# microsoft/AI2BMD

Measured on NVIDIA H100. Metric: MD steps/sec, higher is better.
Workload: dtype f32

## Files before the change

ai2bmd_b200/csrc/engine.cu:

```cuda
#include <cuda_runtime.h>
#include <cxxabi.h>

#include <algorithm>
#include <atomic>
#include <cmath>
#include <cstdarg>
#include <cstdio>
#include <cstdlib>
#include <cstring>
#include <mutex>
#include <string>
#include <vector>

#include "../../include/visnet_b200.h"
#include "k_edge.cuh"
#include "k_caph.cuh"
#include "k_comm.cuh"
#include "k_edge_tc.cuh"
#include "k_graph_embed.cuh"
#include <nvtx3/nvToolsExt.h>
#include "k_head.cuh"
#include "k_md.cuh"
#include "k_nonbonded.cuh"
#include "k_node.cuh"
// ... 572 lines not shown
    a.tile_rows = h->tile_rows;
    const int rows = h->tc_rows;
    const int tiles = (h->ws.Ecap + h->tile_rows - 1) / h->tile_rows;
    const int blocks = std::max(1, std::min(tiles, h->sm_count));
    if (rows == 32) Lc.launch(edge_fwd_tc_kernel<32>, dim3(blocks), dim3(TC2_THREADS), TC_SMEM_BYTES, a);
    else if (rows == 64) Lc.launch(edge_fwd_tc_kernel<64>, dim3(blocks), dim3(TC2_THREADS), TC_SMEM_BYTES, a);
    else if (rows == 96) Lc.launch(edge_fwd_tc_kernel<96>, dim3(blocks), dim3(TC2_THREADS), TC_SMEM_BYTES, a);
    else Lc.launch(edge_fwd_tc_kernel<128>, dim3(blocks), dim3(TC2_THREADS), TC_SMEM_BYTES, a);
    Lc.check();
}

void edge_fwd(Launcher& Lc, int l) {
    if (Lc.h->edge_tc & 1) { launch_edge_fwd_tc(Lc, l); return; }
    if (Lc.h->te_fwd == 64) launch_edge_fwd<64, 8>(Lc, l, 2);
    else launch_edge_fwd<32, 8>(Lc, l, 4);
}
void launch_edge_bwd_tc(Launcher& Lc, int l) {
    vb_handle* h = Lc.h;
    EdgeTcArgs a{};
    a.layer = l; a.mw = h->mw; a.ws = h->ws;
    const LayerW& lw = h->mw.layer[l];
    const size_t chunk = 4 * 8192;
    const bool upd = l < L - 1;
    int n = 0;
    a.jobs[n++] = TcJob{lw.tcWsN, 0};
    a.jobs[n++] = TcJob{lw.tcWsN + chunk, 1};
    a.jobs[n++] = TcJob{lw.tcW1N + chunk, 0};
    a.jobs[n++] = TcJob{lw.tcW1N, 1};
    if (upd) a.jobs[n++] = TcJob{lw.tcW1N + 2 * chunk, 1};
    a.njobs = n;
    a.tl = h->timeline ? h->d_tl + (size_t)(L + l) * TC_TL_SLOTS : nullptr;
    a.tile_rows = h->tile_rows;
    const int rows = h->tc_rows;
    const int tiles = (h->ws.Ecap + h->tile_rows - 1) / h->tile_rows;
    const int blocks = std::max(1, std::min(tiles, h->sm_count));
    if (rows == 32) Lc.launch(edge_bwd_tc_kernel<32>, dim3(blocks), dim3(TC2_THREADS), TC_SMEM_BYTES, a);
    else if (rows == 64) Lc.launch(edge_bwd_tc_kernel<64>, dim3(blocks), dim3(TC2_THREADS), TC_SMEM_BYTES, a);
    else if (rows == 96) Lc.launch(edge_bwd_tc_kernel<96>, dim3(blocks), dim3(TC2_THREADS), TC_SMEM_BYTES, a);
    else Lc.launch(edge_bwd_tc_kernel<128>, dim3(blocks), dim3(TC2_THREADS), TC_SMEM_BYTES, a);
    Lc.check();
}

void edge_bwd(Launcher& Lc, int l) {
    if (Lc.h->edge_tc & 2) { launch_edge_bwd_tc(Lc, l); return; }
    if (Lc.h->te_bwd == 64) launch_edge_bwd<64, 8>(Lc, l, 1);
    else launch_edge_bwd<32, 8>(Lc, l, 2);
}

void node_tc_common(const vb_handle* h, NodeTcArgs& a, int k) {
    a.layer = k; a.mw = h->mw; a.ws = h->ws;
    a.tx = (h->ws.N + TC_TE - 1) / TC_TE;
    a.tv = (3 * h->ws.N + TC_TE - 1) / TC_TE;
    a.njx = 3; a.njv = 5; a.jx = 1; a.jv = 1;
}
void node_tc_jobs(TcJob* jobs, const float* img, int n) {
    for (int c = 0; c < n; c++) jobs[c] = TcJob{img + (size_t)c * 4 * 8192, 0};
// ... 2789 lines not shown
```

ai2bmd_b200/csrc/k_edge_tc.cuh:

```cuda
#pragma once
#include "k_edge.cuh"
#include "tc_common.cuh"

namespace vb {

constexpr int TC_TE = 128;
constexpr int TC_STAGES = 2;
constexpr int TC_MAX_STAGES = 3;
constexpr int TC_SLABS = D / tc::SLAB_K;
static_assert((TC_SLABS & (TC_SLABS - 1)) == 0, "tc_slab rotates the slab order with a mask: TC_SLABS must be a power of two");
constexpr int TC_MAXJOBS = 12;
constexpr int TC_LT = D + LDS_PAD;
typedef float TcRow[TC_LT];

struct TcJob {
    const float* img;
    int accumulate;
};

struct TcShared {
    alignas(1024) uint8_t ring[TC_STAGES][tc::STAGE_BYTES];
    alignas(16) float tile[TC_TE][TC_LT];
    alignas(16) float abuf[TC_TE][TC_LT];
    EdgeMeta<TC_TE> meta;
// ... 39 lines not shown

constexpr int TC2_CWARPS = 16;
constexpr int TC2_CTHREADS = TC2_CWARPS * 32;
constexpr int TC2_THREADS = TC2_CTHREADS;
constexpr int TC2_NGRP = TC2_CTHREADS / D;

struct EdgeTcArgs {
    int layer;
    ModelW mw;
    Workspace ws;
    TcJob jobs[TC_MAXJOBS];
    int njobs;
    int tile_rows;
    unsigned long long* tl;
};
constexpr int TC_TL_SLOTS = 64;
#define TC_TL(k) do { if (a.tl != nullptr && blockIdx.x == 0 && it == 0 && threadIdx.x == 0) a.tl[k] = (unsigned long long)clock64(); } while (0)

__device__ __forceinline__ void csync() { asm volatile("bar.sync 1, %0;" ::"n"(TC2_CTHREADS) : "memory"); }

constexpr int TC2_WS_THREADS = TC2_CTHREADS / 2;
__device__ __forceinline__ bool tc2_is_mma_warp(int warp) { return ((warp >> 2) & 1) == 0; }
__device__ __forceinline__ void gather_sync() { asm volatile("bar.sync 2, %0;" ::"n"(TC2_WS_THREADS) : "memory"); }
__device__ __forceinline__ void handoff_arrive(int id) { asm volatile("bar.arrive %0, %1;" ::"r"(id), "n"(TC2_CTHREADS) : "memory"); }
__device__ __forceinline__ void handoff_wait(int id) { asm volatile("bar.sync %0, %1;" ::"r"(id), "n"(TC2_CTHREADS) : "memory"); }

template <int ROWS>
struct TcRing {
    static constexpr int NS = tc_nstages(ROWS);
    int next = 0;
};

template <int ROWS>
__device__ __forceinline__ void tc2_setup(TcShared& sh, const TcRing<ROWS>&, const TcJob* jobs, int njobs, int ntiles) {
    constexpr int NS = TcRing<ROWS>::NS;
    if (threadIdx.x == 0) {
        for (int s = 0; s < NS; s++) { tc::mbar_init(&sh.b_full[s], 1); sh.released[s] = 0; }
        tc::mbar_init(&sh.b_tile, TC2_CWARPS);
        sh.jobs = jobs; sh.njobs = njobs; sh.nslabs = ntiles * njobs * TC_SLABS;
        tc::fence_barrier_init();
    }
    __syncthreads();
    if (threadIdx.x == 0)
        for (int k = 0; k < NS; k++) tc_issue<NS>(sh, k);
}

// ... 221 lines not shown
    float* __restrict__ Fout = upd ? ws.F[l + 1] : nullptr;
    const float* __restrict__ QKV = ws.QKV[l];
    const float* __restrict__ VN = ws.VN[l];
    const float* __restrict__ TU = ws.TU[l];
    float* __restrict__ P1 = ws.P1[l];
    float* __restrict__ SP = ws.SP[l];
    float* __restrict__ ATT = ws.ATT[l];
    for (int it = 0; it < my_tiles; it++) {
        const uint32_t tpar = (uint32_t)(it & 1);
        const int e0 = ((int)blockIdx.x + it * (int)gridDim.x) * trows;
        const int nvalid = min(trows, E - e0);
        {
            constexpr int RW = ROWS / TC2_CWARPS;
            const int w0 = warp * RW, wn = max(0, min(RW, nvalid - w0));
            if (lane == 0) {
                if (wn > 0) tc::mbar_arrive_expect_tx(&sh.b_tile, (uint32_t)wn * D * 4);
                else tc::mbar_arrive(&sh.b_tile);
            }
            __syncwarp();
            if (lane < wn) tc::tma_load_1d(&sh.abuf[w0 + lane][0], Fin + (size_t)(e0 + w0 + lane) * D, D * 4, &sh.b_tile);
        }
        load_edge_meta<TC_TE, TC2_CTHREADS>(sh.meta, ws, e0, nvalid);
        if constexpr (SMALL) {
            enum : int { H_DK = 3, H_ATT, H_DV, H_F, H_M, H_EU };
            TcRow* const xb = tc_aux(sh);
            csync();
            if (tc2_is_mma_warp(warp)) {
                tc::mbar_wait(&sh.b_tile, tpar);
                TC_TL(2);
                tc2_mma<ROWS, true>(sh, ring, sh.abuf, acc, a.jobs[J_DK].accumulate, warp, lane, nvalid);
                tc2_acc_to(sh.tile, acc, warp, lane, nvalid);
                handoff_arrive(H_DK);
                TC_TL(4);
                tc2_mma<ROWS, true>(sh, ring, sh.abuf, acc, a.jobs[J_DV].accumulate, warp, lane, nvalid);
                TC_TL(7);
                handoff_wait(H_ATT);
                tc2_acc_to(xb, acc, warp, lane, nvalid);
                handoff_arrive(H_DV);
                TC_TL(8);
                if (upd) {
                    tc2_mma<ROWS, true>(sh, ring, sh.abuf, acc, a.jobs[J_F].accumulate, warp, lane, nvalid);
                    tc2_acc_to(sh.tile, acc, warp, lane, nvalid);
                    handoff_arrive(H_F);
                    TC_TL(11);
                }
                handoff_wait(H_M);
                TC_TL(3);
// ... 217 lines not shown
            TC_TL(15);
            if (threadIdx.x == 0 && it + 1 < my_tiles) {
                const int en = ((int)blockIdx.x + (it + 1) * (int)gridDim.x) * trows;
                tc::tma_prefetch_l2(Fin + (size_t)en * D, (uint32_t)min(trows, E - en) * D * 4);
            }
            tc2_mma(sh, ring, sh.abuf, acc, a.jobs[J_S2].accumulate, warp, lane, nvalid);
            TC_TL(16);
            csync();
            tc2_acc_to(sh.tile, acc, warp, lane, nvalid);
            csync();
            TC_TL(17);
            tc_fwd_s2(sh, ws, lw, SP, sh.tile, e0, nvalid, cch, grp, TC2_NGRP, bnd);
            TC_TL(18);
        }
        csync();
    }
    if (a.tl != nullptr && blockIdx.x == 0 && threadIdx.x == 0) a.tl[31] = (unsigned long long)clock64();
}

}

namespace vb {

template <int ROWS>
__global__ void __launch_bounds__(TC2_THREADS, 1) edge_bwd_tc_kernel(const __grid_constant__ EdgeTcArgs a) {
    pdl_entry();
    extern __shared__ __align__(1024) uint8_t dyn_raw[];
    TcShared& sh = *tc_shared_base(dyn_raw);
    const Workspace& ws = a.ws;
    const int l = a.layer;
    const bool upd = (l < L - 1);
    const int J_G3A = 0, J_G3B = 1, J_G4DV = 2, J_G4DK = 3, J_G4F = 4;
    const int J_LAST = upd ? J_G4F : J_G4DK;
    constexpr int RPW = ROWS / TC2_CWARPS;
    constexpr int RB4 = (RPW % 4 == 0) ? 4 : 2;
    constexpr bool SMALL = ROWS <= 64;
    constexpr int RBM = SMALL ? 2 : RB4;
    const int warp = threadIdx.x >> 5, lane = threadIdx.x & 31, col = lane * 4, hd = lane >> 2;
    const int E = ws.rowptr[ws.N];
    const int trows = min(ROWS, max(16, a.tile_rows));
    const int ntiles_total = (E + trows - 1) / trows;
    const int my_tiles = ((int)blockIdx.x < ntiles_total) ? (ntiles_total - (int)blockIdx.x + (int)gridDim.x - 1) / (int)gridDim.x : 0;
    if (a.tl != nullptr && blockIdx.x == 0 && threadIdx.x == 0) a.tl[0] = (unsigned long long)clock64();
    TcRing<ROWS> ring;
    tc2_setup(sh, ring, a.jobs, a.njobs, my_tiles);
    if (a.tl != nullptr && blockIdx.x == 0 && threadIdx.x == 0) a.tl[1] = (unsigned long long)clock64();

    float acc[32];
    const float* __restrict__ QKV = ws.QKV[l];
    const float* __restrict__ VN = ws.VN[l];
    const float* __restrict__ TU = ws.TU[l];
    const float* __restrict__ P1 = ws.P1[l];
    const float* __restrict__ SP = ws.SP[l];
    const float* __restrict__ ATT = ws.ATT[l];
    const int cch = threadIdx.x & (D - 1), grp = threadIdx.x >> 7;
    for (int it = 0; it < my_tiles; it++) {
        const int e0 = ((int)blockIdx.x + it * (int)gridDim.x) * trows;
        const int nvalid = min(trows, E - e0);
        const int rpw = (nvalid + TC2_CWARPS - 1) / TC2_CWARPS, r0 = warp * rpw;
        load_edge_meta<TC_TE, TC2_CTHREADS>(sh.meta, ws, e0, nvalid);
        csync();
// ... 15 lines not shown
                }
#pragma unroll
                for (int u = 0; u < RB4; u++) {
                    const int row = r0 + rb + u;
                    const bool mine = rb + u < rpw, ok = (mine && row < nvalid);
                    const size_t j3 = (size_t)sh.meta.src[row] * 3;
                    const float4 dd = sh.meta.d[row];
                    const float4 s1 = silu4(sp[u][0]), s2 = silu4(sp[u][1]);
                    const float4 gs1 = gM[u][0] * vn[u][0] + gM[u][1] * vn[u][1] + gM[u][2] * vn[u][2];
                    const float gx_ = warp_sum(hsum4(gM[u][0] * s2)), gy_ = warp_sum(hsum4(gM[u][1] * s2)), gz_ = warp_sum(hsum4(gM[u][2] * s2));
                    if (mine) {
                        st4(&sh.abuf[row][col], ok ? gs1 * dsilu4(sp[u][0]) : f4s(0.f));
                        st4(&sh.tile[row][col], ok ? (gM[u][0] * dd.x + gM[u][1] * dd.y + gM[u][2] * dd.z) * dsilu4(sp[u][1]) : f4s(0.f));
                        if (lane == 0) { sh.eacc[row][1] = gx_; sh.eacc[row][2] = gy_; sh.eacc[row][3] = gz_; }
                    }
                    if (ok) {
                        red4(ws.GVNMSG + (j3 + 0) * D + col, gM[u][0] * s1);
                        red4(ws.GVNMSG + (j3 + 1) * D + col, gM[u][1] * s1);
                        red4(ws.GVNMSG + (j3 + 2) * D + col, gM[u][2] * s1);
                    }
                }
            }
            TC_TL(3);
        } else {
#pragma unroll 1
            for (int rb = 0; rb < RPW; rb += RB4) {
                if (rb >= rpw) break;
                float4 sp[RB4], gM[RB4][3], vn[RB4][3];
#pragma unroll
                for (int u = 0; u < RB4; u++) {
                    const int row = r0 + rb + u;
                    const size_t e = (size_t)(e0 + ((rb + u < rpw && row < nvalid) ? row : 0));
                    const size_t i3 = (size_t)sh.meta.dst[row] * 3, j3 = (size_t)sh.meta.src[row] * 3;
                    sp[u] = ldg4(SP + e * 2 * D + col);
#pragma unroll
                    for (int s = 0; s < 3; s++) { gM[u][s] = ldg4(ws.GVEC + (i3 + s) * D + col); vn[u][s] = ldg4(VN + (j3 + s) * D + col); }
                }
#pragma unroll
                for (int u = 0; u < RB4; u++) {
                    const int row = r0 + rb + u;
                    const bool ok = (rb + u < rpw && row < nvalid);
                    const size_t j3 = (size_t)sh.meta.src[row] * 3;
                    const float4 s1 = silu4(sp[u]);
                    const float4 gs1 = gM[u][0] * vn[u][0] + gM[u][1] * vn[u][1] + gM[u][2] * vn[u][2];
                    if (rb + u < rpw) st4(&sh.abuf[row][col], ok ? gs1 * dsilu4(sp[u]) : f4s(0.f));
                    if (ok) {
// ... 1 lines not shown
                        red4(ws.GVNMSG + (j3 + 1) * D + col, gM[u][1] * s1);
                        red4(ws.GVNMSG + (j3 + 2) * D + col, gM[u][2] * s1);
                    }
                }
            }
            TC_TL(3);
#pragma unroll 4
            for (int r = 0; r < RPW; r++) {
                if (r >= rpw) break;
                const int row = r0 + r;
                const bool ok = (r < rpw && row < nvalid);
                const size_t e = (size_t)(e0 + (ok ? row : 0));
                const size_t i3 = (size_t)sh.meta.dst[row] * 3;
                const float4 dd = sh.meta.d[row];
                const float4 sp = ldg4(SP + e * 2 * D + D + col);
                const float4 s2 = silu4(sp);
                const float4 gM0 = ldg4(ws.GVEC + (i3 + 0) * D + col), gM1 = ldg4(ws.GVEC + (i3 + 1) * D + col),
                             gM2 = ldg4(ws.GVEC + (i3 + 2) * D + col);
                const float gx_ = warp_sum(hsum4(gM0 * s2)), gy_ = warp_sum(hsum4(gM1 * s2)), gz_ = warp_sum(hsum4(gM2 * s2));
                if (lane == 0) { sh.eacc[row][1] = gx_; sh.eacc[row][2] = gy_; sh.eacc[row][3] = gz_; }
                st4(&sh.tile[row][col], ok ? (gM0 * dd.x + gM1 * dd.y + gM2 * dd.z) * dsilu4(sp) : f4s(0.f));
            }
            TC_TL(5);
        }
        csync();
        tc2_mma(sh, ring, sh.abuf, acc, a.jobs[J_G3A].accumulate, warp, lane, nvalid);
        TC_TL(6);
        if constexpr (!SMALL) {
            tc2_tile_to_a(sh, nvalid);
            TC_TL(7);
        }
        tc2_mma(sh, ring, SMALL ? sh.tile : sh.abuf, acc, a.jobs[J_G3B].accumulate, warp, lane, nvalid);
        TC_TL(8);
        csync();
        tc2_acc_to(sh.tile, acc, warp, lane, nvalid);
        csync();
        TC_TL(9);
#pragma unroll 1
        for (int rb = 0; rb < RPW; rb += RBM) {
            if (rb >= rpw) break;
            float4 gxa[RBM], vjr[RBM], pdvr[RBM];
            float avr[RBM];
#pragma unroll
            for (int u = 0; u < RBM; u++) {
                const int row = r0 + rb + u;
                const size_t e = (size_t)(e0 + ((rb + u < rpw && row < nvalid) ? row : 0));
                gxa[u] = load_gxa(ws, (size_t)sh.meta.dst[row], col);
                vjr[u] = ldg4(QKV + (size_t)sh.meta.src[row] * 3 * D + 2 * D + col);
                pdvr[u] = ldg4(P1 + e * 3 * D + D + col);
                avr[u] = (rb + u < rpw && row < nvalid) ? __ldg(ATT + e * H + hd) : 0.f;
            }
#pragma unroll
            for (int u = 0; u < RBM; u++) {
                const int row = r0 + rb + u;
                const bool ok = (rb + u < rpw && row < nvalid);
                const size_t j = sh.meta.src[row];
                const float Ce = sh.meta.C[row];
                const float av = avr[u], sa = silu_(av), A = sa * Ce;
                const bool mine = rb + u < rpw;
                const float4 gm = mine ? ld4(&sh.tile[row][col]) + gxa[u] : f4s(0.f);
                const float4 dv = silu4(pdvr[u]);
                if (mine) st4(&sh.abuf[row][col], ok ? gm * vjr[u] * A * dsilu4(pdvr[u]) : f4s(0.f));
                const float gA = quad_sum(hsum4(gm * vjr[u] * dv));
                if (mine && (lane & 3) == 0) sh.gattn[row][hd] = gA * Ce * dsilu_(av);
                const float gc = warp_sum((lane & 3) == 0 ? gA * sa : 0.f);
                if (mine && lane == 0) sh.eacc[row][0] = gc;
                if (ok) red4(ws.GQKV + j * 3 * D + 2 * D + col, gm * dv * A);
            }
        }
        TC_TL(10);
        csync();
#pragma unroll 1
        for (int rb = 0; rb < RPW; rb += RB4) {
            if (rb >= rpw) break;
            float4 pdkr[RB4], qir[RB4], kjr[RB4];
#pragma unroll
            for (int u = 0; u < RB4; u++) {
                const int row = r0 + rb + u;
                const size_t e = (size_t)(e0 + ((rb + u < rpw && row < nvalid) ? row : 0));
                pdkr[u] = ldg4(P1 + e * 3 * D + col);
                qir[u] = ldg4(QKV + (size_t)sh.meta.dst[row] * 3 * D + col);
                kjr[u] = ldg4(QKV + (size_t)sh.meta.src[row] * 3 * D + D + col);
            }
#pragma unroll
            for (int u = 0; u < RB4; u++) {
                const int row = r0 + rb + u;
                const bool ok = (rb + u < rpw && row < nvalid);
                const size_t j = sh.meta.src[row];
                const float4 dk = silu4(pdkr[u]);
                const float gav = sh.gattn[row][hd];
                if (rb + u < rpw) st4(&sh.tile[row][col], ok ? qir[u] * kjr[u] * gav * dsilu4(pdkr[u]) : f4s(0.f));
                if (SMALL && rb + u < rpw) st4(&tc_aux(sh)[row][col], kjr[u] * dk * gav);
                if (ok) red4(ws.GQKV + j * 3 * D + D + col, qir[u] * dk * gav);
            }
        }
        TC_TL(12);
        csync();
        tc2_mma(sh, ring, sh.abuf, acc, a.jobs[J_G4DV].accumulate, warp, lane, nvalid);
        TC_TL(13);
        if constexpr (!SMALL) {
            tc2_tile_to_a(sh, nvalid);
            TC_TL(14);
            csync();
#pragma unroll 4
            for (int r = 0; r < RPW; r++) {
                if (r >= rpw) break;
                const int row = r0 + r;
                const size_t e = (size_t)(e0 + ((r < rpw && row < nvalid) ? row : 0));
                const float4 dk = silu4(ldg4(P1 + e * 3 * D + col));
                const float4 kj = ldg4(QKV + (size_t)sh.meta.src[row] * 3 * D + D + col);
                st4(&sh.tile[row][col], kj * dk * sh.gattn[row][hd]);
            }
            csync();
        }
        {
            const TcRow* const gqb = SMALL ? tc_aux(sh) : sh.tile;
            const int i_first = sh.meta.dst[0], i_last = sh.meta.dst[nvalid - 1];
            for (int i = i_first + grp; i <= i_last; i += TC2_NGRP) {
                const int q0 = ws.rowptr[i], q1 = ws.rowptr[i + 1];
                const int lo = max(q0, e0) - e0, hi = min(q1, e0 + nvalid) - e0;
                float gq = 0.f;
                for (int r = lo; r < hi; r++) gq += gqb[r][cch];
                if (q0 >= e0 && q1 <= e0 + nvalid) ws.GQKV[(size_t)i * 3 * D + cch] = gq;
                else atomicAdd(ws.GQKV + (size_t)i * 3 * D + cch, gq);
            }
        }
        TC_TL(15);
        if (upd) {
            TcRow* const gpfb = SMALL ? sh.abuf : sh.tile;
            csync();
#pragma unroll 1
            for (int rb = 0; rb < RPW; rb += 2) {
                if (rb >= rpw) break;
                float4 gfr[2], pfr[2], tir[2][3], ujr[2][3];
#pragma unroll
                for (int u = 0; u < 2; u++) {
                    const int row = r0 + rb + u;
                    const bool ok = (rb + u < rpw && row < nvalid);
                    const size_t e = (size_t)(e0 + (ok ? row : 0));
                    const size_t i3 = (size_t)sh.meta.dst[row] * 3, j3 = (size_t)sh.meta.src[row] * 3;
                    gfr[u] = ok ? ld4(ws.GF + e * D + col) : f4s(0.f);
                    pfr[u] = ldg4(P1 + e * 3 * D + 2 * D + col);
#pragma unroll
                    for (int s = 0; s < 3; s++) {
                        tir[u][s] = ldg4(TU + (i3 + s) * 2 * D + col);
                        ujr[u][s] = ldg4(TU + (j3 + s) * 2 * D + D + col);
                    }
                }
#pragma unroll
                for (int u = 0; u < 2; u++) {
                    const int row = r0 + rb + u;
                    const bool ok = (rb + u < rpw && row < nvalid);
                    const size_t e = (size_t)(e0 + (ok ? row : 0));
                    const size_t j3 = (size_t)sh.meta.src[row] * 3;
                    const float4 dd = sh.meta.d[row];
                    const float4 gfn = gfr[u], pf = pfr[u];
                    const float4 fp = silu4(pf);
                    const float dv3[3] = {dd.x, dd.y, dd.z};
                    const float4 a1 = tir[u][0] * dd.x + tir[u][1] * dd.y + tir[u][2] * dd.z;
                    const float4 a2 = ujr[u][0] * dd.x + ujr[u][1] * dd.y + ujr[u][2] * dd.z;
                    float4 w1[3], w2[3];
#pragma unroll
                    for (int s = 0; s < 3; s++) { w1[s] = tir[u][s] - a1 * dv3[s]; w2[s] = ujr[u][s] - a2 * dv3[s]; }
                    const float4 wdot = w1[0] * w2[0] + w1[1] * w2[1] + w1[2] * w2[2];
                    const float4 gwd = gfn * fp;
                    if (rb + u < rpw) {
                        st4(&gpfb[row][col], gfn * wdot * dsilu4(pf));
                        if (SMALL) st4(&tc_aux(sh)[row][col], gwd);
                    }
                    const float4 c1 = gwd * (w2[0] * dd.x + w2[1] * dd.y + w2[2] * dd.z);
                    const float4 c2 = gwd * (w1[0] * dd.x + w1[1] * dd.y + w1[2] * dd.z);
                    float gdl[3];
                    float4 gu[3];
#pragma unroll
                    for (int s = 0; s < 3; s++) {
                        const float4 gw1 = gwd * w2[s], gw2 = gwd * w1[s];
                        gu[s] = gw2 - c2 * dv3[s];
                        gdl[s] = warp_sum(hsum4(tir[u][s] * c1 + a1 * gw1 + ujr[u][s] * c2 + a2 * gw2));
                    }
                    if (lane == 0 && rb + u < rpw) { sh.eacc[row][1] -= gdl[0]; sh.eacc[row][2] -= gdl[1]; sh.eacc[row][3] -= gdl[2]; }
                    if (ok) {
                        red4(ws.GTU + (j3 + 0) * 2 * D + D + col, gu[0]);
                        red4(ws.GTU + (j3 + 1) * 2 * D + D + col, gu[1]);
                        red4(ws.GTU + (j3 + 2) * 2 * D + D + col, gu[2]);
                    }
                    (void)e;
                }
            }
            TC_TL(16);
            csync();
            tc2_mma(sh, ring, SMALL ? sh.tile : sh.abuf, acc, a.jobs[J_G4DK].accumulate, warp, lane, nvalid);
            TC_TL(17);
            if constexpr (!SMALL) {
                tc2_tile_to_a(sh, nvalid);
                TC_TL(18);
                csync();
#pragma unroll 4
                for (int r = 0; r < RPW; r++) {
                    if (r >= rpw) break;
                    const int row = r0 + r;
                    const bool ok = (r < rpw && row < nvalid);
                    const size_t e = (size_t)(e0 + (ok ? row : 0));
                    const float4 gfn = ok ? ld4(ws.GF + e * D + col) : f4s(0.f);
                    st4(&sh.tile[row][col], gfn * silu4(ldg4(P1 + e * 3 * D + 2 * D + col)));
                }
                csync();
            }
            {
                const TcRow* const gwb = SMALL ? tc_aux(sh) : sh.tile;
                const int i_first = sh.meta.dst[0], i_last = sh.meta.dst[nvalid - 1];
                for (int i = i_first + grp; i <= i_last; i += TC2_NGRP) {
                    const int q0 = ws.rowptr[i], q1 = ws.rowptr[i + 1];
                    const int lo = max(q0, e0) - e0, hi = min(q1, e0 + nvalid) - e0;
                    float gt0 = 0.f, gt1 = 0.f, gt2 = 0.f;
                    auto term = [&](int r, float u0, float u1, float u2) {
                        const float4 dd = sh.meta.d[r];
                        const float gw = gwb[r][cch];
                        const float a2 = u0 * dd.x + u1 * dd.y + u2 * dd.z;
                        const float w20 = u0 - a2 * dd.x, w21 = u1 - a2 * dd.y, w22 = u2 - a2 * dd.z;
                        const float wd = w20 * dd.x + w21 * dd.y + w22 * dd.z;
                        gt0 += gw * (w20 - wd * dd.x);
                        gt1 += gw * (w21 - wd * dd.y);
                        gt2 += gw * (w22 - wd * dd.z);
                    };
                    int r = lo;
                    for (; r + 4 <= hi; r += 4) {
                        float u[4][3];
#pragma unroll
                        for (int q = 0; q < 4; q++) {
                            const size_t j3 = (size_t)sh.meta.src[r + q] * 3;
                            u[q][0] = __ldg(TU + (j3 + 0) * 2 * D + D + cch);
                            u[q][1] = __ldg(TU + (j3 + 1) * 2 * D + D + cch);
                            u[q][2] = __ldg(TU + (j3 + 2) * 2 * D + D + cch);
                        }
#pragma unroll
                        for (int q = 0; q < 4; q++) term(r + q, u[q][0], u[q][1], u[q][2]);
                    }
                    for (; r < hi; r++) {
                        const size_t j3 = (size_t)sh.meta.src[r] * 3;
                        term(r, __ldg(TU + (j3 + 0) * 2 * D + D + cch), __ldg(TU + (j3 + 1) * 2 * D + D + cch),
                             __ldg(TU + (j3 + 2) * 2 * D + D + cch));
                    }
                    if (q0 >= e0 && q1 <= e0 + nvalid) {
                        ws.GTU[((size_t)i * 3 + 0) * 2 * D + cch] = gt0;
                        ws.GTU[((size_t)i * 3 + 1) * 2 * D + cch] = gt1;
                        ws.GTU[((size_t)i * 3 + 2) * 2 * D + cch] = gt2;
                    } else {
                        atomicAdd(ws.GTU + ((size_t)i * 3 + 0) * 2 * D + cch, gt0);
                        atomicAdd(ws.GTU + ((size_t)i * 3 + 1) * 2 * D + cch, gt1);
                        atomicAdd(ws.GTU + ((size_t)i * 3 + 2) * 2 * D + cch, gt2);
                    }
                }
            }
        }
        TC_TL(19);
        if (threadIdx.x < 3 && it + 1 < my_tiles) {
            const int en = ((int)blockIdx.x + (it + 1) * (int)gridDim.x) * trows;
            const uint32_t nn = (uint32_t)min(trows, E - en);
            if (threadIdx.x == 0) tc::tma_prefetch_l2(SP + (size_t)en * 2 * D, nn * 2 * D * 4);
            else if (threadIdx.x == 1) tc::tma_prefetch_l2(P1 + (size_t)en * 3 * D, nn * 3 * D * 4);
            else tc::tma_prefetch_l2(ATT + (size_t)en * H, nn * H * 4);
        }
        tc2_mma(sh, ring, (SMALL && !upd) ? sh.tile : sh.abuf, acc, a.jobs[J_LAST].accumulate, warp, lane, nvalid);
        TC_TL(20);
        if (!SMALL || !upd) csync();
        tc2_acc_to(sh.tile, acc, warp, lane, nvalid);
        csync();
        TC_TL(21);
#pragma unroll 4
        for (int r = 0; r < RPW; r++) {
            if (r >= rpw) break;
            const int row = r0 + r;
            if ((r < rpw && row < nvalid)) {
                float* g = ws.GF + (size_t)(e0 + row) * D + col;
                float4 v = ld4(&sh.tile[row][col]);
                if (upd) v = v + ld4(g);
                st4(g, v);
            }
        }
        if (threadIdx.x < nvalid) {
            float* ea = ws.eacc + (size_t)(e0 + threadIdx.x) * 4;
            st4(ea, ld4(ea) + ld4(&sh.eacc[threadIdx.x][0]));
        }
        TC_TL(22);
        csync();
    }
    if (a.tl != nullptr && blockIdx.x == 0 && threadIdx.x == 0) a.tl[31] = (unsigned long long)clock64();
}

// ... 2 lines not shown
```

Measured before the change: 1155.

## Warp-specialize small-tile edge backward kernel to overlap MMA with gather work

```diff
diff --git a/ai2bmd_b200/csrc/engine.cu b/ai2bmd_b200/csrc/engine.cu
--- a/ai2bmd_b200/csrc/engine.cu
+++ b/ai2bmd_b200/csrc/engine.cu
@@ -618,16 +618,18 @@
     const LayerW& lw = h->mw.layer[l];
     const size_t chunk = 4 * 8192;
     const bool upd = l < L - 1;
+    const int rows = h->tc_rows;
+    const bool pf_first = upd && rows <= 64;
     int n = 0;
     a.jobs[n++] = TcJob{lw.tcWsN, 0};
     a.jobs[n++] = TcJob{lw.tcWsN + chunk, 1};
-    a.jobs[n++] = TcJob{lw.tcW1N + chunk, 0};
+    if (pf_first) a.jobs[n++] = TcJob{lw.tcW1N + 2 * chunk, 0};
+    a.jobs[n++] = TcJob{lw.tcW1N + chunk, pf_first ? 1 : 0};
     a.jobs[n++] = TcJob{lw.tcW1N, 1};
-    if (upd) a.jobs[n++] = TcJob{lw.tcW1N + 2 * chunk, 1};
+    if (upd && !pf_first) a.jobs[n++] = TcJob{lw.tcW1N + 2 * chunk, 1};
     a.njobs = n;
     a.tl = h->timeline ? h->d_tl + (size_t)(L + l) * TC_TL_SLOTS : nullptr;
     a.tile_rows = h->tile_rows;
-    const int rows = h->tc_rows;
     const int tiles = (h->ws.Ecap + h->tile_rows - 1) / h->tile_rows;
     const int blocks = std::max(1, std::min(tiles, h->sm_count));
     if (rows == 32) Lc.launch(edge_bwd_tc_kernel<32>, dim3(blocks), dim3(TC2_THREADS), TC_SMEM_BYTES, a);
diff --git a/ai2bmd_b200/csrc/k_edge_tc.cuh b/ai2bmd_b200/csrc/k_edge_tc.cuh
--- a/ai2bmd_b200/csrc/k_edge_tc.cuh
+++ b/ai2bmd_b200/csrc/k_edge_tc.cuh
@@ -85,6 +85,7 @@
 constexpr int TC2_WS_THREADS = TC2_CTHREADS / 2;
 __device__ __forceinline__ bool tc2_is_mma_warp(int warp) { return ((warp >> 2) & 1) == 0; }
 __device__ __forceinline__ void gather_sync() { asm volatile("bar.sync 2, %0;" ::"n"(TC2_WS_THREADS) : "memory"); }
+__device__ __forceinline__ void mma_sync() { asm volatile("bar.sync 3, %0;" ::"n"(TC2_WS_THREADS) : "memory"); }
 __device__ __forceinline__ void handoff_arrive(int id) { asm volatile("bar.arrive %0, %1;" ::"r"(id), "n"(TC2_CTHREADS) : "memory"); }
 __device__ __forceinline__ void handoff_wait(int id) { asm volatile("bar.sync %0, %1;" ::"r"(id), "n"(TC2_CTHREADS) : "memory"); }
 
@@ -352,7 +353,7 @@
         }
         load_edge_meta<TC_TE, TC2_CTHREADS>(sh.meta, ws, e0, nvalid);
         if constexpr (SMALL) {
-            enum : int { H_DK = 3, H_ATT, H_DV, H_F, H_M, H_EU };
+            enum : int { H_DK = 4, H_ATT, H_DV, H_F, H_M, H_EU };
             TcRow* const xb = tc_aux(sh);
             csync();
             if (tc2_is_mma_warp(warp)) {
@@ -616,6 +617,202 @@
 
 namespace vb {
 
+
+template <int NR, int RB, class Wait>
+__device__ __forceinline__ void tc_bwd_gm(TcShared& sh, const Workspace& ws, const float* __restrict__ QKV,
+                                          const float* __restrict__ P1, const float* __restrict__ ATT, int e0, int nvalid,
+                                          int r0, int rpw, int lane, Wait&& wait) {
+    const int col = lane * 4, hd = lane >> 2;
+#pragma unroll 1
+    for (int rb = 0; rb < NR; rb += RB) {
+        if (rb >= rpw) break;
+        float4 gxa[RB], vjr[RB], pdvr[RB];
+        float avr[RB];
+#pragma unroll
+        for (int u = 0; u < RB; u++) {
+            const int row = r0 + rb + u;
+            const size_t e = (size_t)(e0 + ((rb + u < rpw && row < nvalid) ? row : 0));
+            gxa[u] = load_gxa(ws, (size_t)sh.meta.dst[row], col);
+            vjr[u] = ldg4(QKV + (size_t)sh.meta.src[row] * 3 * D + 2 * D + col);
+            pdvr[u] = ldg4(P1 + e * 3 * D + D + col);
+            avr[u] = (rb + u < rpw && row < nvalid) ? __ldg(ATT + e * H + hd) : 0.f;
+        }
+        if (rb == 0) wait();
+#pragma unroll
+        for (int u = 0; u < RB; u++) {
+            const int row = r0 + rb + u;
+            const bool ok = (rb + u < rpw && row < nvalid);
+            const size_t j = sh.meta.src[row];
+            const float Ce = sh.meta.C[row];
+            const float av = avr[u], sa = silu_(av), A = sa * Ce;
+            const bool mine = rb + u < rpw;
+            const float4 gm = mine ? ld4(&sh.tile[row][col]) + gxa[u] : f4s(0.f);
+            const float4 dv = silu4(pdvr[u]);
+            if (mine) st4(&sh.abuf[row][col], ok ? gm * vjr[u] * A * dsilu4(pdvr[u]) : f4s(0.f));
+            const float gA = quad_sum(hsum4(gm * vjr[u] * dv));
+            if (mine && (lane & 3) == 0) sh.gattn[row][hd] = gA * Ce * dsilu_(av);
+            const float gc = warp_sum((lane & 3) == 0 ? gA * sa : 0.f);
+            if (mine && lane == 0) sh.eacc[row][0] = gc;
+            if (ok) red4(ws.GQKV + j * 3 * D + 2 * D + col, gm * dv * A);
+        }
+    }
+}
+
+template <int NR, int RB, bool GQ>
+__device__ __forceinline__ void tc_bwd_gpdk(TcShared& sh, const Workspace& ws, const float* __restrict__ QKV,
+                                            const float* __restrict__ P1, int e0, int nvalid, int r0, int rpw, int lane) {
+    const int col = lane * 4, hd = lane >> 2;
+#pragma unroll 1
+    for (int rb = 0; rb < NR; rb += RB) {
+        if (rb >= rpw) break;
+        float4 pdkr[RB], qir[RB], kjr[RB];
+#pragma unroll
+        for (int u = 0; u < RB; u++) {
+            const int row = r0 + rb + u;
+            const size_t e = (size_t)(e0 + ((rb + u < rpw && row < nvalid) ? row : 0));
+            pdkr[u] = ldg4(P1 + e * 3 * D + col);
+            qir[u] = ldg4(QKV + (size_t)sh.meta.dst[row] * 3 * D + col);
+            kjr[u] = ldg4(QKV + (size_t)sh.meta.src[row] * 3 * D + D + col);
+        }
+#pragma unroll
+        for (int u = 0; u < RB; u++) {
+            const int row = r0 + rb + u;
+            const bool ok = (rb + u < rpw && row < nvalid);
+            const size_t j = sh.meta.src[row];
+            const float4 dk = silu4(pdkr[u]);
+            const float gav = sh.gattn[row][hd];
+            if (rb + u < rpw) st4(&sh.tile[row][col], ok ? qir[u] * kjr[u] * gav * dsilu4(pdkr[u]) : f4s(0.f));
+            if (GQ && rb + u < rpw) st4(&tc_aux(sh)[row][col], kjr[u] * dk * gav);
+            if (ok) red4(ws.GQKV + j * 3 * D + D + col, qir[u] * dk * gav);
+        }
+    }
+}
+
+template <int NR>
+__device__ __forceinline__ void tc_bwd_gpf(TcShared& sh, const Workspace& ws, const float* __restrict__ TU,
+                                           const float* __restrict__ P1, TcRow* dst, int e0, int nvalid, int r0, int rpw,
+                                           int lane) {
+    const int col = lane * 4;
+#pragma unroll 1
+    for (int rb = 0; rb < NR; rb += 2) {
+        if (rb >= rpw) break;
+        float4 gfr[2], pfr[2], tir[2][3], ujr[2][3];
+#pragma unroll
+        for (int u = 0; u < 2; u++) {
+            const int row = r0 + rb + u;
+            const bool ok = (rb + u < rpw && row < nvalid);
+            const size_t e = (size_t)(e0 + (ok ? row : 0));
+            const size_t i3 = (size_t)sh.meta.dst[row] * 3, j3 = (size_t)sh.meta.src[row] * 3;
+            gfr[u] = ok ? ld4(ws.GF + e * D + col) : f4s(0.f);
+            pfr[u] = ldg4(P1 + e * 3 * D + 2 * D + col);
+#pragma unroll
+            for (int s = 0; s < 3; s++) {
+                tir[u][s] = ldg4(TU + (i3 + s) * 2 * D + col);
+                ujr[u][s] = ldg4(TU + (j3 + s) * 2 * D + D + col);
+            }
+        }
+#pragma unroll
+        for (int u = 0; u < 2; u++) {
+            const int row = r0 + rb + u;
+            const bool ok = (rb + u < rpw && row < nvalid);
+            const size_t j3 = (size_t)sh.meta.src[row] * 3;
+            const float4 dd = sh.meta.d[row];
+            const float4 gfn = gfr[u], pf = pfr[u];
+            const float4 fp = silu4(pf);
+            const float dv3[3] = {dd.x, dd.y, dd.z};
+            const float4 a1 = tir[u][0] * dd.x + tir[u][1] * dd.y + tir[u][2] * dd.z;
+            const float4 a2 = ujr[u][0] * dd.x + ujr[u][1] * dd.y + ujr[u][2] * dd.z;
+            float4 w1[3], w2[3];
+#pragma unroll
+            for (int s = 0; s < 3; s++) { w1[s] = tir[u][s] - a1 * dv3[s]; w2[s] = ujr[u][s] - a2 * dv3[s]; }
+            const float4 wdot = w1[0] * w2[0] + w1[1] * w2[1] + w1[2] * w2[2];
+            const float4 gwd = gfn * fp;
+            if (rb + u < rpw) st4(&dst[row][col], gfn * wdot * dsilu4(pf));
+            const float4 c1 = gwd * (w2[0] * dd.x + w2[1] * dd.y + w2[2] * dd.z);
+            const float4 c2 = gwd * (w1[0] * dd.x + w1[1] * dd.y + w1[2] * dd.z);
+            float gdl[3];
+            float4 gu[3];
+#pragma unroll
+            for (int s = 0; s < 3; s++) {
+                const float4 gw1 = gwd * w2[s], gw2 = gwd * w1[s];
+                gu[s] = gw2 - c2 * dv3[s];
+                gdl[s] = warp_sum(hsum4(tir[u][s] * c1 + a1 * gw1 + ujr[u][s] * c2 + a2 * gw2));
+            }
+            if (lane == 0 && rb + u < rpw) { sh.eacc[row][1] -= gdl[0]; sh.eacc[row][2] -= gdl[1]; sh.eacc[row][3] -= gdl[2]; }
+            if (ok) {
+                red4(ws.GTU + (j3 + 0) * 2 * D + D + col, gu[0]);
+                red4(ws.GTU + (j3 + 1) * 2 * D + D + col, gu[1]);
+                red4(ws.GTU + (j3 + 2) * 2 * D + D + col, gu[2]);
+            }
+        }
+    }
+}
+
+__device__ __forceinline__ void tc_bwd_gq_sums(const TcShared& sh, const Workspace& ws, const TcRow* gqb, int e0, int nvalid,
+                                               int c, int grp, int ngrp) {
+    const int i_first = sh.meta.dst[0], i_last = sh.meta.dst[nvalid - 1];
+    for (int i = i_first + grp; i <= i_last; i += ngrp) {
+        const int q0 = ws.rowptr[i], q1 = ws.rowptr[i + 1];
+        const int lo = max(q0, e0) - e0, hi = min(q1, e0 + nvalid) - e0;
+        float gq = 0.f;
+        for (int r = lo; r < hi; r++) gq += gqb[r][c];
+        if (q0 >= e0 && q1 <= e0 + nvalid) ws.GQKV[(size_t)i * 3 * D + c] = gq;
+        else atomicAdd(ws.GQKV + (size_t)i * 3 * D + c, gq);
+    }
+}
+template <bool STAGED>
+__device__ __forceinline__ void tc_bwd_gwdot_sums(const TcShared& sh, const Workspace& ws, const float* __restrict__ TU,
+                                                  const float* __restrict__ P1, const TcRow* gwb, int e0, int nvalid, int c,
+                                                  int grp, int ngrp) {
+    const int i_first = sh.meta.dst[0], i_last = sh.meta.dst[nvalid - 1];
+    auto gwd = [&](int r) -> float {
+        if constexpr (STAGED) return gwb[r][c];
+        else return ws.GF[(size_t)(e0 + r) * D + c] * silu_(__ldg(P1 + (size_t)(e0 + r) * 3 * D + 2 * D + c));
+    };
+    for (int i = i_first + grp; i <= i_last; i += ngrp) {
+        const int q0 = ws.rowptr[i], q1 = ws.rowptr[i + 1];
+        const int lo = max(q0, e0) - e0, hi = min(q1, e0 + nvalid) - e0;
+        float gt0 = 0.f, gt1 = 0.f, gt2 = 0.f;
+        auto term = [&](int r, float gw, float u0, float u1, float u2) {
+            const float4 dd = sh.meta.d[r];
+            const float a2 = u0 * dd.x + u1 * dd.y + u2 * dd.z;
+            const float w20 = u0 - a2 * dd.x, w21 = u1 - a2 * dd.y, w22 = u2 - a2 * dd.z;
+            const float wd = w20 * dd.x + w21 * dd.y + w22 * dd.z;
+            gt0 += gw * (w20 - wd * dd.x);
+            gt1 += gw * (w21 - wd * dd.y);
+            gt2 += gw * (w22 - wd * dd.z);
+        };
+        int r = lo;
+        for (; r + 4 <= hi; r += 4) {
+            float u[4][3], gw[4];
+#pragma unroll
+            for (int q = 0; q < 4; q++) {
+                const size_t j3 = (size_t)sh.meta.src[r + q] * 3;
+                u[q][0] = __ldg(TU + (j3 + 0) * 2 * D + D + c);
+                u[q][1] = __ldg(TU + (j3 + 1) * 2 * D + D + c);
+                u[q][2] = __ldg(TU + (j3 + 2) * 2 * D + D + c);
+                gw[q] = gwd(r + q);
+            }
+#pragma unroll
+            for (int q = 0; q < 4; q++) term(r + q, gw[q], u[q][0], u[q][1], u[q][2]);
+        }
+        for (; r < hi; r++) {
+            const size_t j3 = (size_t)sh.meta.src[r] * 3;
+            term(r, gwd(r), __ldg(TU + (j3 + 0) * 2 * D + D + c), __ldg(TU + (j3 + 1) * 2 * D + D + c),
+                 __ldg(TU + (j3 + 2) * 2 * D + D + c));
+        }
+        if (q0 >= e0 && q1 <= e0 + nvalid) {
+            ws.GTU[((size_t)i * 3 + 0) * 2 * D + c] = gt0;
+            ws.GTU[((size_t)i * 3 + 1) * 2 * D + c] = gt1;
+            ws.GTU[((size_t)i * 3 + 2) * 2 * D + c] = gt2;
+        } else {
+            atomicAdd(ws.GTU + ((size_t)i * 3 + 0) * 2 * D + c, gt0);
+            atomicAdd(ws.GTU + ((size_t)i * 3 + 1) * 2 * D + c, gt1);
+            atomicAdd(ws.GTU + ((size_t)i * 3 + 2) * 2 * D + c, gt2);
+        }
+    }
+}
+
 template <int ROWS>
 __global__ void __launch_bounds__(TC2_THREADS, 1) edge_bwd_tc_kernel(const __grid_constant__ EdgeTcArgs a) {
     pdl_entry();
@@ -624,13 +821,12 @@
     const Workspace& ws = a.ws;
     const int l = a.layer;
     const bool upd = (l < L - 1);
-    const int J_G3A = 0, J_G3B = 1, J_G4DV = 2, J_G4DK = 3, J_G4F = 4;
-    const int J_LAST = upd ? J_G4F : J_G4DK;
     constexpr int RPW = ROWS / TC2_CWARPS;
     constexpr int RB4 = (RPW % 4 == 0) ? 4 : 2;
     constexpr bool SMALL = ROWS <= 64;
-    constexpr int RBM = SMALL ? 2 : RB4;
-    const int warp = threadIdx.x >> 5, lane = threadIdx.x & 31, col = lane * 4, hd = lane >> 2;
+    const int J_G3A = 0, J_G3B = 1;
+    const int J_G4F = SMALL ? 2 : 4, J_G4DV = (SMALL && upd) ? 3 : 2, J_G4DK = J_G4DV + 1;
+    const int warp = threadIdx.x >> 5, lane = threadIdx.x & 31, col = lane * 4;
     const int E = ws.rowptr[ws.N];
     const int trows = min(ROWS, max(16, a.tile_rows));
     const int ntiles_total = (E + trows - 1) / trows;
@@ -692,6 +888,70 @@
                 }
             }
             TC_TL(3);
+            csync();
+            enum : int { H_GM = 4, H_PF, H_AUX, H_PDV, H_PDK };
+            TcRow* const xb = tc_aux(sh);
+            constexpr int GRPW = ROWS / (TC2_CWARPS / 2), MRPW = GRPW / 4 > 0 ? GRPW / 4 : 1;
+            constexpr int RBG = GRPW >= 8 ? 3 : 2;
+            const int slice = (warp >> 3) * 4 + (warp & 3);
+            if (tc2_is_mma_warp(warp)) {
+                auto mrow0 = [&] { const int g = (nvalid + 7) / 8; return (((int)threadIdx.x >> 8) * 4 + (((int)threadIdx.x >> 5) & 3) + 1) * g - g / 4; };
+                auto mrows = [&] { return ((nvalid + 7) / 8) / 4; };
+                tc2_mma<ROWS, true>(sh, ring, sh.abuf, acc, a.jobs[J_G3A].accumulate, warp, lane, nvalid);
+                TC_TL(6);
+                tc2_mma<ROWS, true>(sh, ring, sh.tile, acc, a.jobs[J_G3B].accumulate, warp, lane, nvalid);
+                TC_TL(8);
+                mma_sync();
+                tc2_acc_to(sh.tile, acc, warp, lane, nvalid);
+                handoff_arrive(H_GM);
+                mma_sync();
+                TC_TL(9);
+                tc_bwd_gm<MRPW, MRPW >= 2 ? 2 : 1>(sh, ws, QKV, P1, ATT, e0, nvalid, mrow0(), mrows(), lane, [] {});
+                __syncwarp();
+                if (upd) {
+                    handoff_wait(H_PF);
+                    TC_TL(10);
+                    tc2_mma<ROWS, true>(sh, ring, xb, acc, a.jobs[J_G4F].accumulate, warp, lane, nvalid);
+                    handoff_arrive(H_AUX);
+                    TC_TL(11);
+                }
+                handoff_wait(H_PDV);
+                TC_TL(12);
+                tc2_mma<ROWS, true>(sh, ring, sh.abuf, acc, a.jobs[J_G4DV].accumulate, warp, lane, nvalid);
+                TC_TL(13);
+                tc_bwd_gpdk<MRPW, MRPW >= 2 ? 2 : 1, true>(sh, ws, QKV, P1, e0, nvalid, mrow0(), mrows(), lane);
+                if (threadIdx.x < 3 && it + 1 < my_tiles) {
+                    const int en = ((int)blockIdx.x + (it + 1) * (int)gridDim.x) * trows;
+                    const uint32_t nn = (uint32_t)min(trows, E - en);
+                    if (threadIdx.x == 0) tc::tma_prefetch_l2(SP + (size_t)en * 2 * D, nn * 2 * D * 4);
+                    else if (threadIdx.x == 1) tc::tma_prefetch_l2(P1 + (size_t)en * 3 * D, nn * 3 * D * 4);
+                    else tc::tma_prefetch_l2(ATT + (size_t)en * H, nn * H * 4);
+                }
+                handoff_wait(H_PDK);
+                TC_TL(14);
+                tc2_mma<ROWS, true>(sh, ring, sh.tile, acc, a.jobs[J_G4DK].accumulate, warp, lane, nvalid);
+                TC_TL(17);
+            } else {
+                const int grpw = (nvalid + 7) / 8, g0 = slice * grpw, gn = grpw - grpw / 4, gt = slice * 32 + lane;
+                const int gch = gt & (D - 1), ggrp = gt >> 7;
+                if (upd) {
+                    tc_bwd_gpf<GRPW>(sh, ws, TU, P1, xb, e0, nvalid, g0, grpw, lane);
+                    handoff_arrive(H_PF);
+                    TC_TLG(0);
+                }
+                tc_bwd_gm<GRPW, RBG>(sh, ws, QKV, P1, ATT, e0, nvalid, g0, gn, lane,
+                                     [] { handoff_wait(H_GM); });
+                handoff_arrive(H_PDV);
+                __syncwarp();
+                TC_TLG(2);
+                if (upd) handoff_wait(H_AUX);
+                TC_TLG(3);
+                tc_bwd_gpdk<GRPW, RBG, true>(sh, ws, QKV, P1, e0, nvalid, g0, gn, lane);
+                handoff_wait(H_PDK);
+                TC_TLG(4);
+                tc_bwd_gq_sums(sh, ws, xb, e0, nvalid, gch, ggrp, 2);
+                TC_TLG(5);
+            }
         } else {
 #pragma unroll 1
             for (int rb = 0; rb < RPW; rb += RB4) {
@@ -739,83 +999,25 @@
                 st4(&sh.tile[row][col], ok ? (gM0 * dd.x + gM1 * dd.y + gM2 * dd.z) * dsilu4(sp) : f4s(0.f));
             }
             TC_TL(5);
-        }
-        csync();
-        tc2_mma(sh, ring, sh.abuf, acc, a.jobs[J_G3A].accumulate, warp, lane, nvalid);
-        TC_TL(6);
-        if constexpr (!SMALL) {
+            csync();
+            tc2_mma(sh, ring, sh.abuf, acc, a.jobs[J_G3A].accumulate, warp, lane, nvalid);
+            TC_TL(6);
             tc2_tile_to_a(sh, nvalid);
             TC_TL(7);
-        }
-        tc2_mma(sh, ring, SMALL ? sh.tile : sh.abuf, acc, a.jobs[J_G3B].accumulate, warp, lane, nvalid);
-        TC_TL(8);
-        csync();
-        tc2_acc_to(sh.tile, acc, warp, lane, nvalid);
-        csync();
-        TC_TL(9);
-#pragma unroll 1
-        for (int rb = 0; rb < RPW; rb += RBM) {
-            if (rb >= rpw) break;
-            float4 gxa[RBM], vjr[RBM], pdvr[RBM];
-            float avr[RBM];
-#pragma unroll
-            for (int u = 0; u < RBM; u++) {
-                const int row = r0 + rb + u;
-                const size_t e = (size_t)(e0 + ((rb + u < rpw && row < nvalid) ? row : 0));
-                gxa[u] = load_gxa(ws, (size_t)sh.meta.dst[row], col);
-                vjr[u] = ldg4(QKV + (size_t)sh.meta.src[row] * 3 * D + 2 * D + col);
-                pdvr[u] = ldg4(P1 + e * 3 * D + D + col);
-                avr[u] = (rb + u < rpw && row < nvalid) ? __ldg(ATT + e * H + hd) : 0.f;
-            }
-#pragma unroll
-            for (int u = 0; u < RBM; u++) {
-                const int row = r0 + rb + u;
-                const bool ok = (rb + u < rpw && row < nvalid);
-                const size_t j = sh.meta.src[row];
-                const float Ce = sh.meta.C[row];
-                const float av = avr[u], sa = silu_(av), A = sa * Ce;
-                const bool mine = rb + u < rpw;
-                const float4 gm = mine ? ld4(&sh.tile[row][col]) + gxa[u] : f4s(0.f);
-                const float4 dv = silu4(pdvr[u]);
-                if (mine) st4(&sh.abuf[row][col], ok ? gm * vjr[u] * A * dsilu4(pdvr[u]) : f4s(0.f));
-                const float gA = quad_sum(hsum4(gm * vjr[u] * dv));
-                if (mine && (lane & 3) == 0) sh.gattn[row][hd] = gA * Ce * dsilu_(av);
-                const float gc = warp_sum((lane & 3) == 0 ? gA * sa : 0.f);
-                if (mine && lane == 0) sh.eacc[row][0] = gc;
-                if (ok) red4(ws.GQKV + j * 3 * D + 2 * D + col, gm * dv * A);
-            }
-        }
-        TC_TL(10);
-        csync();
-#pragma unroll 1
-        for (int rb = 0; rb < RPW; rb += RB4) {
-            if (rb >= rpw) break;
-            float4 pdkr[RB4], qir[RB4], kjr[RB4];
-#pragma unroll
-            for (int u = 0; u < RB4; u++) {
-                const int row = r0 + rb + u;
-                const size_t e = (size_t)(e0 + ((rb + u < rpw && row < nvalid) ? row : 0));
-                pdkr[u] = ldg4(P1 + e * 3 * D + col);
-                qir[u] = ldg4(QKV + (size_t)sh.meta.dst[row] * 3 * D + col);
-                kjr[u] = ldg4(QKV + (size_t)sh.meta.src[row] * 3 * D + D + col);
-            }
-#pragma unroll
-            for (int u = 0; u < RB4; u++) {
-                const int row = r0 + rb + u;
-                const bool ok = (rb + u < rpw && row < nvalid);
-                const size_t j = sh.meta.src[row];
-                const float4 dk = silu4(pdkr[u]);
-                const float gav = sh.gattn[row][hd];
-                if (rb + u < rpw) st4(&sh.tile[row][col], ok ? qir[u] * kjr[u] * gav * dsilu4(pdkr[u]) : f4s(0.f));
-                if (SMALL && rb + u < rpw) st4(&tc_aux(sh)[row][col], kjr[u] * dk * gav);
-                if (ok) red4(ws.GQKV + j * 3 * D + D + col, qir[u] * dk * gav);
-            }
-        }
-        TC_TL(12);
-        csync();
-        tc2_mma(sh, ring, sh.abuf, acc, a.jobs[J_G4DV].accumulate, warp, lane, nvalid);
-        TC_TL(13);
-        if constexpr (!SMALL) {
+            tc2_mma(sh, ring, sh.abuf, acc, a.jobs[J_G3B].accumulate, warp, lane, nvalid);
+            TC_TL(8);
+            csync();
+            tc2_acc_to(sh.tile, acc, warp, lane, nvalid);
+            csync();
+            TC_TL(9);
+            tc_bwd_gm<RPW, RB4>(sh, ws, QKV, P1, ATT, e0, nvalid, r0, rpw, lane, [] {});
+            TC_TL(10);
+            csync();
+            tc_bwd_gpdk<RPW, RB4, false>(sh, ws, QKV, P1, e0, nvalid, r0, rpw, lane);
+            TC_TL(12);
+            csync();
+            tc2_mma(sh, ring, sh.abuf, acc, a.jobs[J_G4DV].accumulate, warp, lane, nvalid);
+            TC_TL(13);
             tc2_tile_to_a(sh, nvalid);
             TC_TL(14);
             csync();
@@ -826,89 +1028,18 @@
                 const size_t e = (size_t)(e0 + ((r < rpw && row < nvalid) ? row : 0));
                 const float4 dk = silu4(ldg4(P1 + e * 3 * D + col));
                 const float4 kj = ldg4(QKV + (size_t)sh.meta.src[row] * 3 * D + D + col);
-                st4(&sh.tile[row][col], kj * dk * sh.gattn[row][hd]);
-            }
-            csync();
-        }
-        {
-            const TcRow* const gqb = SMALL ? tc_aux(sh) : sh.tile;
-            const int i_first = sh.meta.dst[0], i_last = sh.meta.dst[nvalid - 1];
-            for (int i = i_first + grp; i <= i_last; i += TC2_NGRP) {
-                const int q0 = ws.rowptr[i], q1 = ws.rowptr[i + 1];
-                const int lo = max(q0, e0) - e0, hi = min(q1, e0 + nvalid) - e0;
-                float gq = 0.f;
-                for (int r = lo; r < hi; r++) gq += gqb[r][cch];
-                if (q0 >= e0 && q1 <= e0 + nvalid) ws.GQKV[(size_t)i * 3 * D + cch] = gq;
-                else atomicAdd(ws.GQKV + (size_t)i * 3 * D + cch, gq);
-            }
-        }
-        TC_TL(15);
-        if (upd) {
-            TcRow* const gpfb = SMALL ? sh.abuf : sh.tile;
-            csync();
-#pragma unroll 1
-            for (int rb = 0; rb < RPW; rb += 2) {
-                if (rb >= rpw) break;
-                float4 gfr[2], pfr[2], tir[2][3], ujr[2][3];
-#pragma unroll
-                for (int u = 0; u < 2; u++) {
-                    const int row = r0 + rb + u;
-                    const bool ok = (rb + u < rpw && row < nvalid);
-                    const size_t e = (size_t)(e0 + (ok ? row : 0));
-                    const size_t i3 = (size_t)sh.meta.dst[row] * 3, j3 = (size_t)sh.meta.src[row] * 3;
-                    gfr[u] = ok ? ld4(ws.GF + e * D + col) : f4s(0.f);
-                    pfr[u] = ldg4(P1 + e * 3 * D + 2 * D + col);
-#pragma unroll
-                    for (int s = 0; s < 3; s++) {
-                        tir[u][s] = ldg4(TU + (i3 + s) * 2 * D + col);
-                        ujr[u][s] = ldg4(TU + (j3 + s) * 2 * D + D + col);
-                    }
-                }
-#pragma unroll
-                for (int u = 0; u < 2; u++) {
-                    const int row = r0 + rb + u;
-                    const bool ok = (rb + u < rpw && row < nvalid);
-                    const size_t e = (size_t)(e0 + (ok ? row : 0));
-                    const size_t j3 = (size_t)sh.meta.src[row] * 3;
-                    const float4 dd = sh.meta.d[row];
-                    const float4 gfn = gfr[u], pf = pfr[u];
-                    const float4 fp = silu4(pf);
-                    const float dv3[3] = {dd.x, dd.y, dd.z};
-                    const float4 a1 = tir[u][0] * dd.x + tir[u][1] * dd.y + tir[u][2] * dd.z;
-                    const float4 a2 = ujr[u][0] * dd.x + ujr[u][1] * dd.y + ujr[u][2] * dd.z;
-                    float4 w1[3], w2[3];
-#pragma unroll
-                    for (int s = 0; s < 3; s++) { w1[s] = tir[u][s] - a1 * dv3[s]; w2[s] = ujr[u][s] - a2 * dv3[s]; }
-                    const float4 wdot = w1[0] * w2[0] + w1[1] * w2[1] + w1[2] * w2[2];
-                    const float4 gwd = gfn * fp;
-                    if (rb + u < rpw) {
-                        st4(&gpfb[row][col], gfn * wdot * dsilu4(pf));
-                        if (SMALL) st4(&tc_aux(sh)[row][col], gwd);
-                    }
-                    const float4 c1 = gwd * (w2[0] * dd.x + w2[1] * dd.y + w2[2] * dd.z);
-                    const float4 c2 = gwd * (w1[0] * dd.x + w1[1] * dd.y + w1[2] * dd.z);
-                    float gdl[3];
-                    float4 gu[3];
-#pragma unroll
-                    for (int s = 0; s < 3; s++) {
-                        const float4 gw1 = gwd * w2[s], gw2 = gwd * w1[s];
-                        gu[s] = gw2 - c2 * dv3[s];
-                        gdl[s] = warp_sum(hsum4(tir[u][s] * c1 + a1 * gw1 + ujr[u][s] * c2 + a2 * gw2));
-                    }
-                    if (lane == 0 && rb + u < rpw) { sh.eacc[row][1] -= gdl[0]; sh.eacc[row][2] -= gdl[1]; sh.eacc[row][3] -= gdl[2]; }
-                    if (ok) {
-                        red4(ws.GTU + (j3 + 0) * 2 * D + D + col, gu[0]);
-                        red4(ws.GTU + (j3 + 1) * 2 * D + D + col, gu[1]);
-                        red4(ws.GTU + (j3 + 2) * 2 * D + D + col, gu[2]);
-                    }
-                    (void)e;
-                }
-            }
-            TC_TL(16);
-            csync();
-            tc2_mma(sh, ring, SMALL ? sh.tile : sh.abuf, acc, a.jobs[J_G4DK].accumulate, warp, lane, nvalid);
-            TC_TL(17);
-            if constexpr (!SMALL) {
+                st4(&sh.tile[row][col], kj * dk * sh.gattn[row][lane >> 2]);
+            }
+            csync();
+            tc_bwd_gq_sums(sh, ws, sh.tile, e0, nvalid, cch, grp, TC2_NGRP);
+            TC_TL(15);
+            if (upd) {
+                csync();
+                tc_bwd_gpf<RPW>(sh, ws, TU, P1, sh.tile, e0, nvalid, r0, rpw, lane);
+                TC_TL(16);
+                csync();
+                tc2_mma(sh, ring, sh.abuf, acc, a.jobs[J_G4DK].accumulate, warp, lane, nvalid);
+                TC_TL(17);
                 tc2_tile_to_a(sh, nvalid);
                 TC_TL(18);
                 csync();
@@ -922,66 +1053,25 @@
                     st4(&sh.tile[row][col], gfn * silu4(ldg4(P1 + e * 3 * D + 2 * D + col)));
                 }
                 csync();
-            }
-            {
-                const TcRow* const gwb = SMALL ? tc_aux(sh) : sh.tile;
-                const int i_first = sh.meta.dst[0], i_last = sh.meta.dst[nvalid - 1];
-                for (int i = i_first + grp; i <= i_last; i += TC2_NGRP) {
-                    const int q0 = ws.rowptr[i], q1 = ws.rowptr[i + 1];
-                    const int lo = max(q0, e0) - e0, hi = min(q1, e0 + nvalid) - e0;
-                    float gt0 = 0.f, gt1 = 0.f, gt2 = 0.f;
-                    auto term = [&](int r, float u0, float u1, float u2) {
-                        const float4 dd = sh.meta.d[r];
-                        const float gw = gwb[r][cch];
-                        const float a2 = u0 * dd.x + u1 * dd.y + u2 * dd.z;
-                        const float w20 = u0 - a2 * dd.x, w21 = u1 - a2 * dd.y, w22 = u2 - a2 * dd.z;
-                        const float wd = w20 * dd.x + w21 * dd.y + w22 * dd.z;
-                        gt0 += gw * (w20 - wd * dd.x);
-                        gt1 += gw * (w21 - wd * dd.y);
-                        gt2 += gw * (w22 - wd * dd.z);
-                    };
-                    int r = lo;
-                    for (; r + 4 <= hi; r += 4) {
-                        float u[4][3];
-#pragma unroll
-                        for (int q = 0; q < 4; q++) {
-                            const size_t j3 = (size_t)sh.meta.src[r + q] * 3;
-                            u[q][0] = __ldg(TU + (j3 + 0) * 2 * D + D + cch);
-                            u[q][1] = __ldg(TU + (j3 + 1) * 2 * D + D + cch);
-                            u[q][2] = __ldg(TU + (j3 + 2) * 2 * D + D + cch);
-                        }
-#pragma unroll
-                        for (int q = 0; q < 4; q++) term(r + q, u[q][0], u[q][1], u[q][2]);
-                    }
-                    for (; r < hi; r++) {
-                        const size_t j3 = (size_t)sh.meta.src[r] * 3;
-                        term(r, __ldg(TU + (j3 + 0) * 2 * D + D + cch), __ldg(TU + (j3 + 1) * 2 * D + D + cch),
-                             __ldg(TU + (j3 + 2) * 2 * D + D + cch));
-                    }
-                    if (q0 >= e0 && q1 <= e0 + nvalid) {
-                        ws.GTU[((size_t)i * 3 + 0) * 2 * D + cch] = gt0;
-                        ws.GTU[((size_t)i * 3 + 1) * 2 * D + cch] = gt1;
-                        ws.GTU[((size_t)i * 3 + 2) * 2 * D + cch] = gt2;
-                    } else {
-                        atomicAdd(ws.GTU + ((size_t)i * 3 + 0) * 2 * D + cch, gt0);
-                        atomicAdd(ws.GTU + ((size_t)i * 3 + 1) * 2 * D + cch, gt1);
-                        atomicAdd(ws.GTU + ((size_t)i * 3 + 2) * 2 * D + cch, gt2);
-                    }
-                }
-            }
-        }
-        TC_TL(19);
-        if (threadIdx.x < 3 && it + 1 < my_tiles) {
-            const int en = ((int)blockIdx.x + (it + 1) * (int)gridDim.x) * trows;
-            const uint32_t nn = (uint32_t)min(trows, E - en);
-            if (threadIdx.x == 0) tc::tma_prefetch_l2(SP + (size_t)en * 2 * D, nn * 2 * D * 4);
-            else if (threadIdx.x == 1) tc::tma_prefetch_l2(P1 + (size_t)en * 3 * D, nn * 3 * D * 4);
-            else tc::tma_prefetch_l2(ATT + (size_t)en * H, nn * H * 4);
-        }
-        tc2_mma(sh, ring, (SMALL && !upd) ? sh.tile : sh.abuf, acc, a.jobs[J_LAST].accumulate, warp, lane, nvalid);
-        TC_TL(20);
-        if (!SMALL || !upd) csync();
-        tc2_acc_to(sh.tile, acc, warp, lane, nvalid);
+                tc_bwd_gwdot_sums<true>(sh, ws, TU, P1, sh.tile, e0, nvalid, cch, grp, TC2_NGRP);
+            }
+            TC_TL(19);
+            if (threadIdx.x < 3 && it + 1 < my_tiles) {
+                const int en = ((int)blockIdx.x + (it + 1) * (int)gridDim.x) * trows;
+                const uint32_t nn = (uint32_t)min(trows, E - en);
+                if (threadIdx.x == 0) tc::tma_prefetch_l2(SP + (size_t)en * 2 * D, nn * 2 * D * 4);
+                else if (threadIdx.x == 1) tc::tma_prefetch_l2(P1 + (size_t)en * 3 * D, nn * 3 * D * 4);
+                else tc::tma_prefetch_l2(ATT + (size_t)en * H, nn * H * 4);
+            }
+            tc2_mma(sh, ring, sh.abuf, acc, a.jobs[upd ? J_G4F : J_G4DK].accumulate, warp, lane, nvalid);
+            TC_TL(20);
+        }
+        csync();
+        if (!SMALL || tc2_is_mma_warp(warp)) tc2_acc_to(sh.tile, acc, warp, lane, nvalid);
+        if (SMALL && upd) {
+            tc_bwd_gwdot_sums<false>(sh, ws, TU, P1, nullptr, e0, nvalid, cch, grp, TC2_NGRP);
+            TC_TL(19);
+        }
         csync();
         TC_TL(21);
 #pragma unroll 4
```

After: 1178 (median of 6 runs). 2.0% higher.
